# SandeepaInduwaraSamaranayake/SwinVox

Measured on AMD Instinct MI355X. Metric: views/sec fwd+bwd SwinVox-T 224^2, 32^3 voxel, n_views=8, higher is better.
Workload: dtype bf16; 1 GPU; SwinVox-T full pipeline (ResNet50[:layer3] || Swin multi-stage, cross-view attention, decoder, merger, refiner), fwd+2xBCE+bwd, train mode, B=64 samples x V=8 views of 224x224 per GPU; global_batch=64, n_views=8, images_per_gpu=512, parallelism=single GPU, launch=eager (one host launch per kernel, three streams)

## Files before the change

swinvox_amd/csrc/stencil.hip:

```cpp
#include "common.h"
#include <map>
#include <mutex>
#include <type_traits>

namespace sv {

constexpr int TZ = 4, TY = 8, TX = 8;
constexpr int HZ = TZ + 2, HY = TY + 2, HX = TX + 2;
constexpr int HPOS = HZ * HY * HX;
constexpr int NVOX = TZ * TY * TX;
typedef __attribute__((address_space(3))) bf16x4 lds_bf16x4_t;

__device__ __forceinline__ bf16x4 to_bf16x4(float4 v) {
  bf16x4 b;
  b[0] = (__bf16)v.x; b[1] = (__bf16)v.y; b[2] = (__bf16)v.z; b[3] = (__bf16)v.w;
  return b;
}
__device__ __forceinline__ bf16x4 to_bf16x4(bf16x4 v) { return v; }

__device__ __forceinline__ int xcd_first_tile() {
  const int n = gridDim.x, b = blockIdx.x;
  return (n & 7) == 0 ? (b & 7) * (n >> 3) + (b >> 3) : b;
}

struct TileId { int img, z0, y0, x0; };
template <int TZV = TZ>
__device__ __forceinline__ TileId tile_of(int t, int D, int H, int W) {
  const int tz = D / TZV, ty = H / TY, tx = W / TX;
  TileId r;
  r.x0 = (t % tx) * TX; t /= tx; r.y0 = (t % ty) * TY; t /= ty; r.z0 = (t % tz) * TZV; r.img = t / tz;
  return r;
}

template <int G, typename AT, int TZV = TZ, int NTHR = 256>
struct HaloRegs {
  static constexpr int HZV = TZV + 2, HPOSV = HZV * HY * HX;
  static constexpr int C = 16 * G, VPP = C / 4, N = (HPOSV * VPP + NTHR - 1) / NTHR;
  typedef typename std::conditional<G == 1, int, long long>::type OffT;
  typename V4<AT>::type r[N];
  OffT off[N];
  int face[N];
  int lds[N];
  __device__ __forceinline__ void init(int ldx, long long plane, int cin_load, int H, int W, int tid, int pitch = HX) {
#pragma unroll
    for (int k = 0; k < N; ++k) {
      const int i = tid + NTHR * k;
      const int h = i / VPP, v = i - h * VPP;
      const int hx = h % HX; const int t2 = h / HX; const int hy = t2 % HY; const int hz = t2 / HY;
      const int cv = v * 4, pl = plane ? cv / ldx : 0;
      face[k] = (hz == 0 ? 1 : 0) | (hz == HZV - 1 ? 2 : 0) | (hy == 0 ? 4 : 0) | (hy == HY - 1 ? 8 : 0) | (hx == 0 ? 16 : 0) | (hx == HX - 1 ? 32 : 0) |
                ((i < HPOSV * VPP && cv < cin_load) ? 0 : 64);
      off[k] = (OffT)pl * (OffT)plane + (OffT)(((hz * H + hy) * W + hx) * ldx + (cv - pl * ldx));
      lds[k] = ((hz * HY + hy) * pitch + hx) * C + cv;
    }
  }
  __device__ __forceinline__ void load(const AT* __restrict__ x, int ldx, const TileId& t, int D, int H, int W) {
    const int out = (t.z0 == 0 ? 1 : 0) | (t.z0 + TZV == D ? 2 : 0) | (t.y0 == 0 ? 4 : 0) | (t.y0 + TY == H ? 8 : 0) | (t.x0 == 0 ? 16 : 0) | (t.x0 + TX == W ? 32 : 0) | 64;
    const AT* corner = x + ((((long long)t.img * D + t.z0 - 1) * H + t.y0 - 1) * W + t.x0 - 1) * (long long)ldx;
#pragma unroll
    for (int k = 0; k < N; ++k) {
      typename V4<AT>::type q = V4<AT>::zero();
#ifndef SV_ST_PROBE_NOLOAD
      if ((face[k] & out) == 0) q = V4<AT>::load(corner + off[k]);
#endif
      r[k] = q;
    }
  }
  __device__ __forceinline__ void store(__bf16* Xs, int tid) const {
#pragma unroll
    for (int k = 0; k < N; ++k) {
      const int i = tid + NTHR * k;
      if (i < HPOSV * VPP) *reinterpret_cast<bf16x4*>(Xs + lds[k]) = to_bf16x4(r[k]);
    }
  }
};

template <int G, typename AT, int TZV, int NTHR>
struct HaloSliceRegs {
  static constexpr int HZV = TZV + 2, C = 16 * G, VPP = C / 4;
  static constexpr int ZG = G == 1 ? 5 : 2, NGRP = HZV / ZG, GV = ZG * HY * HX * VPP, NP = (GV + NTHR - 1) / NTHR, N = NGRP * NP;
  static_assert(HZV % ZG == 0, "groups of whole z-slices");
  static_assert(HZV * HY * 16 * C < (1 << 20), "LDS offsets (pitch <= 16 positions) take 20 bits");
  typename V4<AT>::type r[N];
  int off[NP], meta[NP];
  long long plane_;
  int gstep_, lstep_;
  __device__ __forceinline__ void init(int ldx, long long plane, int cin_load, int H, int W, int tid, int pitch) {
#pragma unroll
    for (int j = 0; j < NP; ++j) {
      const int i = tid + NTHR * j;
      int h = i / VPP, v = i - h * VPP;
      const int nvp = ldx / 4;
      if (plane && VPP % nvp == 0) {
        const int row = i / (HX * VPP), rem = i - row * (HX * VPP);
        const int pq = rem / (HX * nvp), r2 = rem - pq * (HX * nvp), px = r2 / nvp;
        h = row * HX + px; v = pq * nvp + (r2 - px * nvp);
      }
      const int hx = h % HX; const int t2 = h / HX; const int hy = t2 % HY; const int hz = t2 / HY;
      const int cv = v * 4, pl = plane ? cv / ldx : 0;
      const int fc = (hz == 0 ? 1 : 0) | (hz == ZG - 1 ? 2 : 0) | (hy == 0 ? 4 : 0) | (hy == HY - 1 ? 8 : 0) | (hx == 0 ? 16 : 0) | (hx == HX - 1 ? 32 : 0) |
                     ((i < GV && cv < cin_load) ? 0 : 64);
      const int lo = i < GV ? ((hz * HY + hy) * pitch + hx) * C + cv : 0;
      meta[j] = lo | (fc << 20) | (pl << 27);
      off[j] = ((hz * H + hy) * W + hx) * ldx + (cv - pl * ldx);
    }
    plane_ = plane; gstep_ = ZG * H * W * ldx; lstep_ = ZG * HY * pitch * C;
  }
  __device__ __forceinline__ void load(const AT* __restrict__ x, int ldx, const TileId& t, int D, int H, int W) {
    const int zlo = t.z0 == 0 ? 1 : 0, zhi = t.z0 + TZV == D ? 2 : 0;
    const int yx = (t.y0 == 0 ? 4 : 0) | (t.y0 + TY == H ? 8 : 0) | (t.x0 == 0 ? 16 : 0) | (t.x0 + TX == W ? 32 : 0) | 64;
    const AT* corner = x + ((((long long)t.img * D + t.z0 - 1) * H + t.y0 - 1) * W + t.x0 - 1) * (long long)ldx;
#pragma unroll
    for (int g = 0; g < NGRP; ++g) {
      const int out = (yx | (g == 0 ? zlo : 0) | (g == NGRP - 1 ? zhi : 0)) << 20;
      const AT* cg = corner + (long long)g * gstep_;
#pragma unroll
      for (int j = 0; j < NP; ++j) {
        typename V4<AT>::type q = V4<AT>::zero();
#ifndef SV_ST_PROBE_NOLOAD
        if ((meta[j] & out) == 0) {
          if constexpr (G > 1) q = V4<AT>::load(cg + (long long)((meta[j] >> 27) & 15) * plane_ + off[j]);
          else q = V4<AT>::load(cg + off[j]);
        }
#endif
        r[g * NP + j] = q;
      }
    }
  }
  __device__ __forceinline__ void store(__bf16* Xs, int tid) const {
#pragma unroll
    for (int g = 0; g < NGRP; ++g)
#pragma unroll
      for (int j = 0; j < NP; ++j)
        if ((j + 1) * NTHR <= GV || tid + NTHR * j < GV) *reinterpret_cast<bf16x4*>(Xs + g * lstep_ + (meta[j] & 0xfffff)) = to_bf16x4(r[g * NP + j]);
  }
};

template <typename AT>
struct StencilArgsT {
  const AT* x; int ldx; int cin_load;
  long long x_plane, out_plane;
  const __bf16* w;
  const float* bias; AT* out; int ldc; int col_off; int cout;
  const AT* residual; int ldr;
  double* stats;
  int I, D, H, W, ntiles;
};

template <int G> struct StencilPitch { static constexpr int HXP = G == 1 ? 16 : HX; };
template <int G> struct StencilBrick { static constexpr int TZV = 8, NTHR = TZV * 64; };
template <int G> struct StencilBrickF { static constexpr int TZV = 8, NTHR = TZV * 64; };
template <int G, int NT, typename AT, bool VEC>
__global__ __launch_bounds__(StencilBrickF<G>::NTHR, 2) void stencil3_fwd_kernel(const StencilArgsT<AT> p) {
  constexpr int C = 16 * G, KTOT = 27 * C, KPAD = (KTOT + 31) / 32 * 32, NSTEP = KPAD / 32, HXP = StencilPitch<G>::HXP;
  constexpr int TZV = StencilBrickF<G>::TZV, NTHR = StencilBrickF<G>::NTHR, NW = NTHR / 64;
  __shared__ __attribute__((aligned(16))) char xc[(TZV + 2) * HY * HXP * C * 2];
  __shared__ __attribute__((aligned(16))) __bf16 Ws[NT * 16 * KPAD];
  __shared__ float red[16 * 16 * 2];
  __bf16* Xs = reinterpret_cast<__bf16*>(xc);
  const int tid = threadIdx.x, lane = tid & 63, wave = tid >> 6;
  const int lr = lane & 15, lg = lane >> 4;

  for (int i = tid; i < NT * 16 * KPAD / 8; i += NTHR) {
    const int n = (i * 8) / KPAD, k = (i * 8) - n * KPAD;
    bf16x8 v = VecN<__bf16, 8>::zero();
    if (k < KTOT) v = *reinterpret_cast<const bf16x8*>(p.w + (size_t)n * KTOT + k);
    *reinterpret_cast<bf16x8*>(Ws + n * KPAD + k) = v;
  }
  const int cs4 = (p.cout + 3) & ~3;
  float bias4[NT][4], st1[4] = {0.f, 0.f, 0.f, 0.f}, st2[4] = {0.f, 0.f, 0.f, 0.f};
#pragma unroll
  for (int nt = 0; nt < NT; ++nt)
#pragma unroll
    for (int j = 0; j < 4; ++j) { const int n = nt * 16 + lg * 4 + j; bias4[nt][j] = (p.bias && n < p.cout) ? p.bias[n] : 0.f; }

  HaloRegs<G, AT, TZV, NTHR> hr;
  hr.init(p.ldx, p.x_plane, p.cin_load, p.H, p.W, tid, HXP);
  int tile = xcd_first_tile();
  TileId t = tile_of<TZV>(tile < p.ntiles ? tile : 0, p.D, p.H, p.W);
  if (tile < p.ntiles) { hr.load(p.x, p.ldx, t, p.D, p.H, p.W); hr.store(Xs, tid); }
  __syncthreads();
  const int yy = lr >> 3, xx = lr & 7;
  int toff[NSTEP];
#pragma unroll
  for (int s = 0; s < NSTEP; ++s) {
    const int kb = s * 32 + lg * 8;
    int tap = kb / C; const int c = kb - tap * C;
    if (tap > 26) tap = 26;
    const int dz = tap / 9, dy = (tap - dz * 9) / 3, dx = tap - dz * 9 - dy * 3;
    toff[s] = (((dz * HY + dy) * HXP + dx) * C + c) * 2;
  }
  const char* xrow = xc + ((wave * HY + yy) * HXP + xx) * C * 2;
  const char* wrow = reinterpret_cast<const char*>(Ws) + (lr * KPAD + lg * 8) * 2;
  const int n0 = lg * 4;
  bool colreal[NT][4];
#pragma unroll
  for (int nt = 0; nt < NT; ++nt)
#pragma unroll
    for (int j = 0; j < 4; ++j) colreal[nt][j] = nt * 16 + n0 + j < p.cout;
  for (; tile < p.ntiles; tile += gridDim.x) {
    const int next = tile + gridDim.x;
    TileId tn = t;
    if (next < p.ntiles) { tn = tile_of<TZV>(next, p.D, p.H, p.W); hr.load(p.x, p.ldx, tn, p.D, p.H, p.W); }

    f32x4 acc[4][NT];
#pragma unroll
    for (int mt = 0; mt < 4; ++mt)
#pragma unroll
      for (int nt = 0; nt < NT; ++nt) acc[mt][nt] = (f32x4){0.f, 0.f, 0.f, 0.f};
#ifndef SV_ST_PROBE_NOMMA
#pragma unroll
    for (int s = 0; s < NSTEP; ++s) {
      bf16x8 b[NT];
#pragma unroll
      for (int nt = 0; nt < NT; ++nt) b[nt] = *reinterpret_cast<const bf16x8*>(wrow + nt * 16 * KPAD * 2 + s * 64);
      const char* ap = xrow + toff[s];
#pragma unroll
      for (int mt = 0; mt < 4; ++mt) {
        const bf16x8 a = *reinterpret_cast<const bf16x8*>(ap + mt * (2 * HXP * C * 2));
#pragma unroll
        for (int nt = 0; nt < NT; ++nt) acc[mt][nt] = __builtin_amdgcn_mfma_f32_16x16x32_bf16(b[nt], a, acc[mt][nt], 0, 0, 0);
      }
    }
#endif
    const size_t pos0 = (((size_t)t.img * p.D + t.z0 + wave) * p.H + t.y0 + yy) * p.W + t.x0 + xx;
    if constexpr (VEC) {
#pragma unroll
      for (int nt = 0; nt < NT; ++nt) {
        const int nn = nt * 16 + n0;
        if (nn >= cs4) continue;
        AT* orow; const AT* rrow = nullptr;
        if (p.out_plane) { const int pl = nn / p.ldc; orow = p.out + (size_t)pl * p.out_plane + pos0 * p.ldc + (nn - pl * p.ldc); }
        else orow = p.out + pos0 * p.ldc + p.col_off + nn;
        if (p.residual) rrow = p.residual + pos0 * p.ldr + nn;
#pragma unroll
        for (int mt = 0; mt < 4; ++mt) {
          float v[4];
#pragma unroll
          for (int j = 0; j < 4; ++j) v[j] = colreal[nt][j] ? acc[mt][nt][j] + bias4[nt][j] : 0.f;
          if (NT == 1 && p.stats) {
#pragma unroll
            for (int j = 0; j < 4; ++j) { st1[j] += v[j]; st2[j] += v[j] * v[j]; }
          }
          if (p.residual) {
            const float4 rv = ld4f(rrow + (size_t)mt * 2 * p.W * p.ldr);
            v[0] += rv.x; v[1] += rv.y; v[2] += rv.z; v[3] += rv.w;
          }
#ifdef SV_ST_PROBE_NOSTORE
          if (v[0] == 1234.5f)
#endif
          st4f(orow + (size_t)mt * 2 * p.W * p.ldc, make_float4(v[0], v[1], v[2], v[3]));
        }
      }
    } else {
#pragma unroll
      for (int mt = 0; mt < 4; ++mt) {
        const size_t pos = pos0 + (size_t)mt * 2 * p.W;
#pragma unroll
        for (int nt = 0; nt < NT; ++nt) {
          const int nn = nt * 16 + n0;
#pragma unroll
          for (int j = 0; j < 4; ++j) {
            if (nn + j < p.cout) {
              float r = acc[mt][nt][j] + bias4[nt][j];
              if (NT == 1 && p.stats) { st1[j] += r; st2[j] += r * r; }
              if (p.residual) r += ldf(p.residual + pos * p.ldr + nn + j);
              stf(p.out + pos * p.ldc + p.col_off + nn + j, r);
            }
          }
        }
      }
    }
    t = tn;
    __syncthreads();
    if (next < p.ntiles) hr.store(Xs, tid);
    __syncthreads();
  }
  if (NT == 1 && p.stats) {
#pragma unroll
    for (int j = 0; j < 4; ++j) {
      { st1[j] += dpp_move<0xB1>(st1[j]); st1[j] += dpp_move<0x4E>(st1[j]); st1[j] += dpp_move<0x141>(st1[j]); st1[j] += dpp_move<0x140>(st1[j]);
        st2[j] += dpp_move<0xB1>(st2[j]); st2[j] += dpp_move<0x4E>(st2[j]); st2[j] += dpp_move<0x141>(st2[j]); st2[j] += dpp_move<0x140>(st2[j]); }
    }
    if (lr == 0) {
#pragma unroll
      for (int j = 0; j < 4; ++j) { red[(wave * 16 + lg * 4 + j) * 2] = st1[j]; red[(wave * 16 + lg * 4 + j) * 2 + 1] = st2[j]; }
    }
    __syncthreads();
    if (tid < 16 && tid < p.cout) {
      float a = 0.f, b = 0.f;
#pragma unroll
      for (int w = 0; w < NW; ++w) { a += red[(w * 16 + tid) * 2]; b += red[(w * 16 + tid) * 2 + 1]; }
      double* st = p.stats + (size_t)(blockIdx.x % SV_BN_SLOTS) * 2 * p.cout;
      atomicAdd(st + tid, (double)a);
      atomicAdd(st + p.cout + tid, (double)b);
    }
  }
}

template <typename AT>
struct StencilWArgsT {
  const AT* x; int ldx; int cin_load;
  long long x_plane;
  const AT* dy; int lddy; int cout_load;
  float* dw;
  float* ws;
  float* dbias;
  int cout, cin;
  int c_stride, c_valid;
  int I, D, H, W, ntiles;
};

constexpr int WG_SLOTS = 16;
__global__ __launch_bounds__(256) void stencil_wgrad_fold_kernel(const float* __restrict__ ws, float* __restrict__ dw, int n) {
  const int i = blockIdx.x * 256 + threadIdx.x;
  if (i >= n) return;
  float a = 0.f;
#pragma unroll
  for (int sl = 0; sl < WG_SLOTS; ++sl) a += ws[(size_t)sl * n + i];
  dw[i] += a;
}

template <int G, typename AT>
__global__ __launch_bounds__(StencilBrick<G>::NTHR, 2) void stencil3_wgrad_kernel(const StencilWArgsT<AT> p) {
  constexpr int C = 16 * G, TZV = StencilBrick<G>::TZV, NTHR = StencilBrick<G>::NTHR, NW = NTHR / 64, NTAPW = (27 + NW - 1) / NW;
  constexpr int HPOSV = (TZV + 2) * HY * HX, NVOXV = TZV * TY * TX;
  __shared__ __attribute__((aligned(16))) __bf16 Xs[HPOSV * C];
  __shared__ __attribute__((aligned(16))) __bf16 Ds[NVOXV * 16];
  __shared__ float bred[NTHR / 16 * 16];
  const int tid = threadIdx.x, lane = tid & 63, wave = tid >> 6;
  const int lr = lane & 15, lg = lane >> 4, q = lr >> 2, pp = lr & 3;
  const int ntap = (27 - wave + NW - 1) / NW;
  f32x4 acc[NTAPW][G];
#pragma unroll
  for (int i = 0; i < NTAPW; ++i)
#pragma unroll
    for (int gg = 0; gg < G; ++gg) acc[i][gg] = (f32x4){0.f, 0.f, 0.f, 0.f};
  float bsum = 0.f;

  HaloRegs<G, AT, TZV, NTHR> hr;
  hr.init(p.ldx, p.x_plane, p.cin_load, p.H, p.W, tid);
  typename V4<AT>::type dr[4];
  auto load_dy = [&](const TileId& t) {
#pragma unroll
    for (int k = 0; k < 4; ++k) {
      const int i = tid + NTHR * k;
      const int v = i >> 2, c4 = i & 3;
      const int xx = v % TX; const int t2 = v / TX; const int yy = t2 % TY; const int zz = t2 / TY;
      typename V4<AT>::type qv = V4<AT>::zero();
      if (c4 * 4 < p.cout_load)
        qv = V4<AT>::load(p.dy + ((((size_t)t.img * p.D + t.z0 + zz) * p.H + t.y0 + yy) * p.W + t.x0 + xx) * (size_t)p.lddy + c4 * 4);
      dr[k] = qv;
    }
  };
  auto store_dy = [&]() {
#pragma unroll
    for (int k = 0; k < 4; ++k) *reinterpret_cast<bf16x4*>(Ds + (tid + NTHR * k) * 4) = to_bf16x4(dr[k]);
  };

  int tile = xcd_first_tile();
  if (tile < p.ntiles) {
    const TileId t = tile_of<TZV>(tile, p.D, p.H, p.W);
    hr.load(p.x, p.ldx, t, p.D, p.H, p.W); load_dy(t);
    hr.store(Xs, tid); store_dy();
  }
  __syncthreads();
  for (; tile < p.ntiles; tile += gridDim.x) {
    const int next = tile + gridDim.x;
    if (next < p.ntiles) {
      const TileId t = tile_of<TZV>(next, p.D, p.H, p.W);
      hr.load(p.x, p.ldx, t, p.D, p.H, p.W); load_dy(t);
    }
    if (p.dbias) {
      const int c = tid & 15, vg = tid >> 4;
#pragma unroll
      for (int k = 0; k < 16; ++k) bsum += (float)Ds[(vg * 16 + k) * 16 + c];
    }
#pragma unroll 1
    for (int ch = 0; ch < 2 * TZV; ++ch) {
      const int z = ch >> 1, yb = (ch & 1) * 4 + lg;
      const __bf16* asrc = Ds + (((z * TY + yb) * TX) + q) * 16 + pp * 4;
      const bf16x4 alo = __builtin_amdgcn_ds_read_tr16_b64_v4bf16((lds_bf16x4_t*)(asrc));
      const bf16x4 ahi = __builtin_amdgcn_ds_read_tr16_b64_v4bf16((lds_bf16x4_t*)(asrc + 4 * 16));
      const bf16x8 a = __builtin_shufflevector(alo, ahi, 0, 1, 2, 3, 4, 5, 6, 7);
#pragma unroll
      for (int i = 0; i < NTAPW; ++i) {
        if (i < ntap) {
          const int tap = wave + NW * i;
          const int dz = tap / 9, dy = (tap - dz * 9) / 3, dx = tap - dz * 9 - dy * 3;
          const int hb = ((z + dz) * HY + yb + dy) * HX + dx + q;
#pragma unroll
          for (int gg = 0; gg < G; ++gg) {
            const __bf16* bsrc = Xs + hb * C + gg * 16 + pp * 4;
            const bf16x4 blo = __builtin_amdgcn_ds_read_tr16_b64_v4bf16((lds_bf16x4_t*)(bsrc));
            const bf16x4 bhi = __builtin_amdgcn_ds_read_tr16_b64_v4bf16((lds_bf16x4_t*)(bsrc + 4 * C));
            const bf16x8 b = __builtin_shufflevector(blo, bhi, 0, 1, 2, 3, 4, 5, 6, 7);
            acc[i][gg] = __builtin_amdgcn_mfma_f32_16x16x32_bf16(a, b, acc[i][gg], 0, 0, 0);
          }
        }
      }
    }
    __syncthreads();
    if (next < p.ntiles) { hr.store(Xs, tid); store_dy(); }
    __syncthreads();
  }
  if (p.dbias) {
    bred[tid] = bsum;
    __syncthreads();
    if (tid < 16 && tid < p.cout) {
      float a = 0.f;
#pragma unroll
      for (int g2 = 0; g2 < NTHR / 16; ++g2) a += bred[g2 * 16 + tid];
      atomicAdd(p.dbias + tid, a);
    }
  }
  float* dst = p.ws ? p.ws + (size_t)(blockIdx.x % WG_SLOTS) * p.cout * p.cin * 27 : p.dw;
#pragma unroll
  for (int i = 0; i < NTAPW; ++i) {
    if (i < ntap) {
      const int tap = wave + NW * i;
#pragma unroll
      for (int gg = 0; gg < G; ++gg) {
        const int cm = gg * 16 + lr;
        const int grp = cm / p.c_stride, within = cm - grp * p.c_stride;
        const int ci = grp * p.c_valid + within;
        if (within < p.c_valid && ci < p.cin) {
#pragma unroll
          for (int j = 0; j < 4; ++j) {
            const int co = lg * 4 + j;
            if (co < p.cout) atomicAdd(dst + ((size_t)co * p.cin + ci) * 27 + tap, acc[i][gg][j]);
          }
        }
      }
    }
  }
}

#ifdef SV_ST_PROBE_WG_PITCH
constexpr int SWEEP_HXP = SV_ST_PROBE_WG_PITCH;
#else
constexpr int SWEEP_HXP = 12;
#endif
#ifdef SV_ST_PROBE_WG_LA
constexpr int SWEEP_LA = SV_ST_PROBE_WG_LA;
#else
constexpr int SWEEP_LA = 1;
#endif
#ifdef SV_ST_PROBE_WG_NOSWAP
constexpr int SWEEP_DYSWAP = 0;
#else
constexpr int SWEEP_DYSWAP = 4;
#endif
template <int G, typename AT>
__global__ __launch_bounds__(StencilBrick<G>::NTHR, G == 1 && sizeof(AT) == 2 ? 4 : 2) void stencil3_wgrad_sweep_kernel(const StencilWArgsT<AT> p) {
  constexpr int C = 16 * G, TZV = StencilBrick<G>::TZV, NTHR = StencilBrick<G>::NTHR, HXP = SWEEP_HXP;
  constexpr int XELEMS = (TZV + 2) * HY * HXP * C, NVOXV = TZV * TY * TX, LA = SWEEP_LA;
  static_assert(NTHR == 512 && NTHR * 4 == NVOXV * 4, "8 waves: 2 y-halves x 4 pair slots; dy staging = 4 vectors per thread");
  static_assert(4 * 9 * G * 64 * 4 * sizeof(float) <= XELEMS * sizeof(__bf16), "the half-1 accumulators are handed over through the x image");
  __shared__ __attribute__((aligned(16))) __bf16 Xs[XELEMS];
  __shared__ __attribute__((aligned(16))) __bf16 Ds[NVOXV * 16];
  __shared__ float bred[2 * 64];
  const int tid = threadIdx.x, lane = tid & 63, wave = __builtin_amdgcn_readfirstlane(tid >> 6);
  const int lr = lane & 15, lg = lane >> 4, q = lr >> 2, pp = lr & 3;
  const int half = wave & 1, slot = wave >> 1;
  const int p0 = slot ? 1 + 2 * slot : 0;
  const bool three = slot == 0, sums_bias = p.dbias != nullptr && slot == 1;
  f32x4 acc[3][3][G];
#pragma unroll
  for (int pi = 0; pi < 3; ++pi)
#pragma unroll
    for (int dz = 0; dz < 3; ++dz)
#pragma unroll
      for (int gg = 0; gg < G; ++gg) acc[pi][dz][gg] = (f32x4){0.f, 0.f, 0.f, 0.f};
  float bsum = 0.f;

  HaloSliceRegs<G, AT, TZV, NTHR> hr;
  hr.init(p.ldx, p.x_plane, p.cin_load, p.H, p.W, tid, HXP);
  typename V4<AT>::type dr[4];
  const int dv0 = tid >> 2, dc4 = (tid & 3) * 4;
  const int dyoff = (((dv0 / (TY * TX)) * p.H + (dv0 / TX) % TY) * p.W + dv0 % TX) * p.lddy + dc4;
  const int dystep = 2 * p.H * p.W * p.lddy;
  auto load_dy = [&](const TileId& t) {
    const AT* d0 = p.dy + ((((size_t)t.img * p.D + t.z0) * p.H + t.y0) * p.W + t.x0) * (size_t)p.lddy + dyoff;
#pragma unroll
    for (int k = 0; k < 4; ++k) {
      typename V4<AT>::type qv = V4<AT>::zero();
      if (dc4 < p.cout_load) qv = V4<AT>::load(d0 + (size_t)k * dystep);
      dr[k] = qv;
    }
  };
  auto store_dy = [&]() {
#pragma unroll
    for (int k = 0; k < 4; ++k) {
      const int i = tid + NTHR * k;
      const int v = i >> 2, vs = v ^ (((v >> 3) & 1) * SWEEP_DYSWAP);
      *reinterpret_cast<bf16x4*>(Ds + vs * 16 + (i & 3) * 4) = to_bf16x4(dr[k]);
    }
  };
  const int yb = 4 * half + lg;
  const __bf16* xsrc[3];
#pragma unroll
  for (int pi = 0; pi < 3; ++pi) {
    const int pr = (pi < 2 || three) ? p0 + pi : p0;
    const int dy = pr / 3, dx = pr - dy * 3;
    xsrc[pi] = Xs + ((yb + dy) * HXP + dx + q) * C + pp * 4;
  }
  const __bf16* alo_src = Ds + (yb * TX + q + ((yb & 1) ? SWEEP_DYSWAP : 0)) * 16 + pp * 4;
  const __bf16* ahi_src = Ds + (yb * TX + q + 4 - ((yb & 1) ? SWEEP_DYSWAP : 0)) * 16 + pp * 4;

  auto read_dy = [&](int z) {
    const bf16x4 alo = __builtin_amdgcn_ds_read_tr16_b64_v4bf16((lds_bf16x4_t*)(alo_src + z * TY * TX * 16));
    const bf16x4 ahi = __builtin_amdgcn_ds_read_tr16_b64_v4bf16((lds_bf16x4_t*)(ahi_src + z * TY * TX * 16));
    return (bf16x8)__builtin_shufflevector(alo, ahi, 0, 1, 2, 3, 4, 5, 6, 7);
  };
  auto read_x = [&](int s, int pi, int gg) {
    const __bf16* bsrc = xsrc[pi] + s * HY * HXP * C + gg * 16;
    const bf16x4 blo = __builtin_amdgcn_ds_read_tr16_b64_v4bf16((lds_bf16x4_t*)(bsrc));
    const bf16x4 bhi = __builtin_amdgcn_ds_read_tr16_b64_v4bf16((lds_bf16x4_t*)(bsrc + 4 * C));
    return (bf16x8)__builtin_shufflevector(blo, bhi, 0, 1, 2, 3, 4, 5, 6, 7);
  };
  auto sweep = [&](auto PI0, auto NPI) {
    constexpr int pi0 = decltype(PI0)::value, npi = decltype(NPI)::value, NSTEP = (TZV + 2) * npi * G;
    bf16x8 a[4];
    bf16x8 b[LA + 1];
    a[0] = read_dy(0);
#pragma unroll
    for (int n = 0; n < LA; ++n) b[n] = read_x(n / (npi * G), pi0 + (n / G) % npi, n % G);
#pragma unroll
    for (int n = 0; n < NSTEP; ++n) {
      const int s = n / (npi * G), pi = pi0 + (n / G) % npi, gg = n % G;
      if (n % (npi * G) == 0 && s + 1 < TZV) a[(s + 1) % 4] = read_dy(s + 1);
      if (n + LA < NSTEP) b[(n + LA) % (LA + 1)] = read_x((n + LA) / (npi * G), pi0 + ((n + LA) / G) % npi, (n + LA) % G);
      __builtin_amdgcn_sched_barrier(0);
#pragma unroll
      for (int dz = 0; dz < 3; ++dz)
        if (s - dz >= 0 && s - dz < TZV) acc[pi][dz][gg] = __builtin_amdgcn_mfma_f32_16x16x32_bf16(a[(s - dz) % 4], b[n % (LA + 1)], acc[pi][dz][gg], 0, 0, 0);
      __builtin_amdgcn_sched_barrier(0);
    }
  };

  int tile = xcd_first_tile();
  if (tile < p.ntiles) {
    const TileId t = tile_of<TZV>(tile, p.D, p.H, p.W);
    hr.load(p.x, p.ldx, t, p.D, p.H, p.W); load_dy(t);
    hr.store(Xs, tid); store_dy();
  }
  __syncthreads();
  for (; tile < p.ntiles; tile += gridDim.x) {
    const int next = tile + gridDim.x;
    if (next < p.ntiles) {
      const TileId t = tile_of<TZV>(next, p.D, p.H, p.W);
      hr.load(p.x, p.ldx, t, p.D, p.H, p.W); load_dy(t);
    }
#ifndef SV_ST_PROBE_NOMMA
    sweep(std::integral_constant<int, 0>(), std::integral_constant<int, 2>());
    if (three) sweep(std::integral_constant<int, 2>(), std::integral_constant<int, 1>());
    if (sums_bias) {
#pragma unroll
      for (int z = 0; z < TZV; ++z) {
        const bf16x8 a = read_dy(z);
        float t8 = 0.f;
#pragma unroll
        for (int j = 0; j < 8; ++j) t8 += (float)a[j];
        bsum += t8;
      }
    }
#endif
    __syncthreads();
    if (next < p.ntiles) { hr.store(Xs, tid); store_dy(); }
    __syncthreads();
  }
  f32x4* hand = reinterpret_cast<f32x4*>(Xs) + (size_t)slot * 9 * G * 64 + lane;
  if (half == 1) {
#pragma unroll
    for (int pi = 0; pi < 3; ++pi)
#pragma unroll
      for (int dz = 0; dz < 3; ++dz)
#pragma unroll
        for (int gg = 0; gg < G; ++gg) hand[((pi * 3 + dz) * G + gg) * 64] = acc[pi][dz][gg];
  }
  if (sums_bias) bred[half * 64 + lane] = bsum;
  __syncthreads();
  if (p.dbias && tid < 16 && tid < p.cout) {
    float s8 = 0.f;
#pragma unroll
    for (int g2 = 0; g2 < 8; ++g2) s8 += bred[g2 * 16 + tid];
    atomicAdd(p.dbias + tid, s8);
  }
  if (half == 1) return;
  float* dst = p.ws ? p.ws + (size_t)(blockIdx.x % WG_SLOTS) * p.cout * p.cin * 27 : p.dw;
#pragma unroll
  for (int pi = 0; pi < 3; ++pi) {
    if (pi < 2 || three) {
#pragma unroll
      for (int dz = 0; dz < 3; ++dz) {
        const int tap = dz * 9 + p0 + pi;
#pragma unroll
        for (int gg = 0; gg < G; ++gg) {
          const f32x4 o = hand[((pi * 3 + dz) * G + gg) * 64];
          const int cm = gg * 16 + lr;
          const int grp = cm / p.c_stride, within = cm - grp * p.c_stride;
          const int ci = grp * p.c_valid + within;
          if (within < p.c_valid && ci < p.cin) {
#pragma unroll
            for (int j = 0; j < 4; ++j) {
              const int co = lg * 4 + j;
              if (co < p.cout) atomicAdd(dst + ((size_t)co * p.cin + ci) * 27 + tap, acc[pi][dz][gg][j] + o[j]);
            }
          }
        }
      }
    }
  }
}

struct TConv4Args {
  const __bf16* x; const __bf16* w;
  const float* bias; __bf16* out; double* stats; int cout; int I, D, H, W, nbricks;
};
constexpr int T4_JZ = 4, T4_JY = 4, T4_JX = 8, T4_HZ = 6, T4_HY = 6, T4_HX = 10, T4_HPOS = T4_HZ * T4_HY * T4_HX;

__global__ __launch_bounds__(256, 2) void tconv4s2_fwd_kernel(const TConv4Args p) {
  __shared__ __attribute__((aligned(16))) __bf16 Xs[T4_HPOS * 32];
  __shared__ __attribute__((aligned(16))) __bf16 Ws[8 * 8 * 256];
  __shared__ __attribute__((aligned(16))) __bf16 Os[8 * 8 * 16 * 8];
  __shared__ float red[4][16];
  const int tid = threadIdx.x, lane = tid & 63, wave = tid >> 6;
  const int lr = lane & 15, lg = lane >> 4;
  for (int i = tid; i < 8 * 8 * 256 / 8; i += 256) {
    const int c8 = (i & 3) * 8, t = (i >> 2) & 7, co = (i >> 5) & 7, cls = i >> 8;
    const int az = cls >> 2, ay = (cls >> 1) & 1, ax = cls & 1, dz = t >> 2, dy = (t >> 1) & 1, dx = t & 1;
    const int kz = az ? 2 - 2 * dz : 3 - 2 * dz, ky = ay ? 2 - 2 * dy : 3 - 2 * dy, kx = ax ? 2 - 2 * dx : 3 - 2 * dx;
    bf16x8 v = VecN<__bf16, 8>::zero();
    if (co < p.cout) v = *reinterpret_cast<const bf16x8*>(p.w + ((size_t)co * 64 + (kz * 4 + ky) * 4 + kx) * 32 + c8);
    *reinterpret_cast<bf16x8*>(Ws + ((cls * 8 + co) * 256) + t * 32 + c8) = v;
  }
  float bias4[4];
#pragma unroll
  for (int j = 0; j < 4; ++j) bias4[j] = (p.bias && lg < 2 && lg * 4 + j < p.cout) ? p.bias[lg * 4 + j] : 0.f;
  double st1[8], st2[8];
#pragma unroll
  for (int c = 0; c < 8; ++c) { st1[c] = 0.0; st2[c] = 0.0; }
  const int bz = p.D / T4_JZ, by = p.H / T4_JY, bx = p.W / T4_JX;
  __syncthreads();
  for (int brick = blockIdx.x; brick < p.nbricks; brick += gridDim.x) {
    int t = brick;
    const int x0 = (t % bx) * T4_JX; t /= bx;
    const int y0 = (t % by) * T4_JY; t /= by;
    const int z0 = (t % bz) * T4_JZ; const int img = t / bz;
    for (int i = tid; i < T4_HPOS * 4; i += 256) {
      const int h = i >> 2, c8 = (i & 3) * 8;
      const int hx = h % T4_HX; const int t2 = h / T4_HX; const int hy = t2 % T4_HY; const int hz = t2 / T4_HY;
      const int z = z0 - 1 + hz, y = y0 - 1 + hy, xx = x0 - 1 + hx;
      bf16x8 v = VecN<__bf16, 8>::zero();
      if ((unsigned)z < (unsigned)p.D && (unsigned)y < (unsigned)p.H && (unsigned)xx < (unsigned)p.W)
        v = *reinterpret_cast<const bf16x8*>(p.x + ((((size_t)img * p.D + z) * p.H + y) * p.W + xx) * 32 + c8);
      *reinterpret_cast<bf16x8*>(Xs + h * 32 + c8) = v;
    }
    __syncthreads();
    const int yy = lr >> 3, xx = lr & 7;
#pragma unroll 1
    for (int ci = 0; ci < 2; ++ci) {
      const int cls = 2 * wave + ci, az = cls >> 2, ay = (cls >> 1) & 1, ax = cls & 1;
      bf16x8 b[8];
#pragma unroll
      for (int tt = 0; tt < 8; ++tt) {
        b[tt] = VecN<__bf16, 8>::zero();
        if (lr < 8) b[tt] = *reinterpret_cast<const bf16x8*>(Ws + (cls * 8 + lr) * 256 + tt * 32 + lg * 8);
      }
#pragma unroll 2
      for (int g = 0; g < 8; ++g) {
        const int jz = g >> 1, jy = (g & 1) * 2 + yy;
        const int base = ((jz + az) * T4_HY + (jy + ay)) * T4_HX + (xx + ax);
        f32x4 acc = (f32x4){0.f, 0.f, 0.f, 0.f};
#pragma unroll
        for (int tt = 0; tt < 8; ++tt) {
          const int off = ((tt >> 2) * T4_HY + ((tt >> 1) & 1)) * T4_HX + (tt & 1);
          const bf16x8 a = *reinterpret_cast<const bf16x8*>(Xs + (base + off) * 32 + lg * 8);
          acc = __builtin_amdgcn_mfma_f32_16x16x32_bf16(b[tt], a, acc, 0, 0, 0);
        }
        if (lg < 2) {
          bf16x4 o;
#pragma unroll
          for (int j = 0; j < 4; ++j) o[j] = (__bf16)(acc[j] + bias4[j]);
          const int oz = 2 * jz + az, oy = 2 * jy + ay, ox = 2 * xx + ax;
          *reinterpret_cast<bf16x4*>(Os + ((oz * 8 + oy) * 16 + ox) * 8 + lg * 4) = o;
        }
      }
    }
    __syncthreads();
#pragma unroll
    for (int k = 0; k < 4; ++k) {
      const int v = tid + 256 * k;
      const int ox = v & 15, oy = (v >> 4) & 7, oz = v >> 7;
      const bf16x8 o = *reinterpret_cast<const bf16x8*>(Os + v * 8);
      const size_t pos = (((size_t)img * (2 * p.D) + 2 * z0 + oz) * (2 * p.H) + 2 * y0 + oy) * (2 * p.W) + 2 * x0 + ox;
      *reinterpret_cast<bf16x8*>(p.out + pos * 8) = o;
      if (p.stats) {
#pragma unroll
        for (int c = 0; c < 8; ++c) { const double f = (double)(float)o[c]; st1[c] += f; st2[c] += f * f; }
      }
    }
    __syncthreads();
  }
  if (p.stats) {
#pragma unroll
    for (int c = 0; c < 8; ++c) {
      float a = (float)st1[c], b2 = (float)st2[c];
      a = wave_sum(a); b2 = wave_sum(b2);
      if (lane == 0) { red[wave][c] = a; red[wave][8 + c] = b2; }
    }
    __syncthreads();
    if (tid < 16 && (tid & 7) < p.cout) {
      const float v = red[0][tid] + red[1][tid] + red[2][tid] + red[3][tid];
      double* st = p.stats + (size_t)(blockIdx.x % SV_BN_SLOTS) * 2 * p.cout;
      atomicAdd(st + (tid >> 3) * p.cout + (tid & 7), (double)v);
    }
  }
}

}

using namespace sv;

static int resident_per_cu(const void* kernel, int threads = 256) {
  static std::mutex mu;
  static std::map<const void*, int> cache;
  std::lock_guard<std::mutex> lk(mu);
  auto it = cache.find(kernel);
  if (it != cache.end()) return it->second;
  int n = 0;
  if (hipOccupancyMaxActiveBlocksPerMultiprocessor(&n, kernel, threads, 0) != hipSuccess || n < 1) { (void)hipGetLastError(); n = 1; }
  cache[kernel] = n;
  return n;
}

static int stencil_check(int I, int D, int H, int W) {
  SV_REQUIRE(I > 0 && D % 8 == 0 && H % TY == 0 && W % TX == 0, "stencil3: grid %dx%dx%d must be a multiple of the 8x8x8 brick", D, H, W);
  return SV_OK;
}

#define SV_STENCIL_LAUNCH(GG, NTT, VV)                                                                                     \
  do {                                                                                                                    \
    constexpr int nthr = StencilBrickF<GG>::NTHR;                                                                         \
    const int nt_ = I * (D / StencilBrickF<GG>::TZV) * (H / TY) * (W / TX);                                               \
    a.ntiles = nt_;                                                                                                       \
    const int resident = 256 * resident_per_cu((const void*)stencil3_fwd_kernel<GG, NTT, AT, VV>, nthr);                  \
    hipLaunchKernelGGL((stencil3_fwd_kernel<GG, NTT, AT, VV>), dim3(nt_ < resident ? nt_ : resident), dim3(nthr), 0, s, a); \
  } while (0)

extern "C" int sv_stencil3_fwd(const void* x, int ldx, int cin_load, int groups, const void* w_bf16, int ntiles16,
                               const float* bias, void* out, int ldc, int col_off, int cout, const void* residual, int ldr,
                               double* stats, int I, int D, int H, int W, long long x_plane_stride, long long out_plane_stride,
                               int act_dtype, void* stream) {
  SV_REQUIRE(x && w_bf16 && out, "stencil3_fwd: null argument");
  SV_REQUIRE(x_plane_stride >= 0 && out_plane_stride >= 0 && x_plane_stride % 4 == 0 && out_plane_stride % 4 == 0, "stencil3_fwd: bad plane strides");
  SV_REQUIRE(!out_plane_stride || (col_off == 0 && !residual && ldc % 4 == 0 && cout % ldc == 0),
             "stencil3_fwd: planar output needs col_off == 0, no residual and whole planes of ldc (multiple of 4) columns");
  SV_REQUIRE_ACT(act_dtype);
  if (int rc = stencil_check(I, D, H, W)) return rc;
    SV_REQUIRE(cin_load % 4 == 0 && cin_load <= 16 * groups && ldx % 4 == 0 && (x_plane_stride ? cin_load % ldx == 0 : ldx >= cin_load),
             "stencil3_fwd: bad input channels (cin_load=%d ldx=%d groups=%d)", cin_load, ldx, groups);
  SV_REQUIRE(cout > 0 && cout <= 16 * ntiles16 && (out_plane_stride || ldc >= col_off + cout), "stencil3_fwd: bad output window");
  SV_REQUIRE(!stats || ntiles16 == 1, "stencil3_fwd: statistics need a single 16-column tile");
  const uintptr_t amask = act_dtype == SV_BF16 ? 7 : 15;
  SV_REQUIRE(((uintptr_t)x & amask) == 0 && ((uintptr_t)w_bf16 & 15) == 0, "stencil3_fwd: operands must be aligned to 4 elements");
  SV_REQUIRE((ldc & 3) != 0 || (((uintptr_t)out | (uintptr_t)residual) & amask) == 0,
             "stencil3_fwd: out/residual must be aligned to 4 elements when ldc is a multiple of 4");
  const int ntiles = I * (D / TZ) * (H / TY) * (W / TX);
  hipStream_t s = (hipStream_t)stream;
  if (!((groups == 1 && ntiles16 == 1) || (groups == 3 && ntiles16 == 1) || (groups == 1 && ntiles16 == 3))) {
    set_error("stencil3_fwd: unsupported (groups=%d, ntiles16=%d)", groups, ntiles16);
    return SV_ERR_INVALID;
  }
  SV_DISPATCH_ACT(act_dtype,
    const int cs4 = (cout + 3) & ~3;
    const bool vec = out_plane_stride != 0 || ((ldc & 3) == 0 && (col_off & 3) == 0 && col_off + cs4 <= ldc && (!residual || ((ldr & 3) == 0 && cs4 <= ldr)));
    StencilArgsT<AT> a{static_cast<const AT*>(x), ldx, cin_load, x_plane_stride, out_plane_stride, (const __bf16*)w_bf16, bias, static_cast<AT*>(out), ldc, col_off, cout,
                       static_cast<const AT*>(residual), ldr, stats, I, D, H, W, ntiles};
    if (groups == 1 && ntiles16 == 1) { if (vec) SV_STENCIL_LAUNCH(1, 1, true); else SV_STENCIL_LAUNCH(1, 1, false); }
    else if (groups == 3) { if (vec) SV_STENCIL_LAUNCH(3, 1, true); else SV_STENCIL_LAUNCH(3, 1, false); }
    else { if (vec) SV_STENCIL_LAUNCH(1, 3, true); else SV_STENCIL_LAUNCH(1, 3, false); });
  return check_launch("sv_stencil3_fwd");
}

extern "C" size_t sv_stencil3_wgrad_workspace_floats(int cout, int cin) { return (size_t)WG_SLOTS * cout * cin * 27; }

extern "C" int sv_stencil3_wgrad(const void* x, int ldx, int cin_load, int groups, const void* dy, int lddy, int cout_load,
                                 float* dw, float* dbias, float* workspace, int cout, int cin, int c_stride, int c_valid, int I, int D, int H,
                                 int W, long long x_plane_stride, int act_dtype, void* stream) {
  SV_REQUIRE(x && dy && dw, "stencil3_wgrad: null argument");
  SV_REQUIRE(x_plane_stride >= 0 && x_plane_stride % 4 == 0 && (!x_plane_stride || cin_load % ldx == 0), "stencil3_wgrad: bad plane stride");
  SV_REQUIRE_ACT(act_dtype);
  if (int rc = stencil_check(I, D, H, W)) return rc;
  SV_REQUIRE(cin_load % 4 == 0 && cin_load <= 16 * groups && ldx % 4 == 0 && cout_load % 4 == 0 && cout_load <= 16 && lddy % 4 == 0,
             "stencil3_wgrad: bad channel layout");
  SV_REQUIRE(cout > 0 && cout <= 16 && cin > 0 && c_stride > 0 && c_valid > 0, "stencil3_wgrad: bad channel counts");
  SV_REQUIRE((((uintptr_t)x | (uintptr_t)dy) & (act_dtype == SV_BF16 ? 7 : 15)) == 0, "stencil3_wgrad: operands must be aligned to 4 elements");
  SV_REQUIRE(groups == 1 || groups == 3, "stencil3_wgrad: unsupported groups=%d", groups);
    const int ntiles = I * (D / (groups == 3 ? StencilBrick<3>::TZV : StencilBrick<1>::TZV)) * (H / TY) * (W / TX);
  hipStream_t s = (hipStream_t)stream;
  const char* sweep_env = getenv("SV_STENCIL_WGRAD_SWEEP");
  const bool sweep = sweep_env ? atoi(sweep_env) != 0 : true;
  SV_DISPATCH_ACT(act_dtype,
    const void* k1 = sweep ? (const void*)stencil3_wgrad_sweep_kernel<1, AT> : (const void*)stencil3_wgrad_kernel<1, AT>;
    const void* k3 = sweep ? (const void*)stencil3_wgrad_sweep_kernel<3, AT> : (const void*)stencil3_wgrad_kernel<3, AT>;
    const int per_cu = groups == 1 ? resident_per_cu(k1, StencilBrick<1>::NTHR) : resident_per_cu(k3, StencilBrick<3>::NTHR);
    const int resident = 256 * per_cu;
    const int blocks = ntiles < resident ? ntiles : resident;
    StencilWArgsT<AT> a{static_cast<const AT*>(x), ldx, cin_load, x_plane_stride, static_cast<const AT*>(dy), lddy, cout_load, dw, workspace, dbias, cout, cin, c_stride, c_valid,
                        I, D, H, W, ntiles};
    if (groups == 1 && sweep) hipLaunchKernelGGL((stencil3_wgrad_sweep_kernel<1, AT>), dim3(blocks), dim3(StencilBrick<1>::NTHR), 0, s, a);
    else if (groups == 1) hipLaunchKernelGGL((stencil3_wgrad_kernel<1, AT>), dim3(blocks), dim3(StencilBrick<1>::NTHR), 0, s, a);
    else if (sweep) hipLaunchKernelGGL((stencil3_wgrad_sweep_kernel<3, AT>), dim3(blocks), dim3(StencilBrick<3>::NTHR), 0, s, a);
    else hipLaunchKernelGGL((stencil3_wgrad_kernel<3, AT>), dim3(blocks), dim3(StencilBrick<3>::NTHR), 0, s, a););
  if (workspace) hipLaunchKernelGGL(stencil_wgrad_fold_kernel, dim3(cdiv(cout * cin * 27, 256)), dim3(256), 0, s, workspace, dw, cout * cin * 27);
  return check_launch("sv_stencil3_wgrad");
}

extern "C" int sv_tconv4s2_fwd(const void* x, const void* w_packed, const float* bias, void* out, double* stats, int I, int D, int H, int W,
                               int cin, int cout, void* stream) {
  SV_REQUIRE(x && w_packed && out && I > 0, "tconv4s2_fwd: null argument");
  SV_REQUIRE(cin == 32 && cout > 0 && cout <= 8, "tconv4s2_fwd: built for 32 input and <= 8 output channels (got %d -> %d)", cin, cout);
  SV_REQUIRE(D % T4_JZ == 0 && H % T4_JY == 0 && W % T4_JX == 0, "tconv4s2_fwd: input grid %dx%dx%d must be a multiple of the 4x4x8 brick", D, H, W);
  SV_REQUIRE((((uintptr_t)x | (uintptr_t)w_packed | (uintptr_t)out) & 15) == 0, "tconv4s2_fwd: operands must be 16-byte aligned");
  TConv4Args a{static_cast<const __bf16*>(x), static_cast<const __bf16*>(w_packed), bias, static_cast<__bf16*>(out), stats, cout, I, D, H, W,
               I * (D / T4_JZ) * (H / T4_JY) * (W / T4_JX)};
  const int blocks = a.nbricks < 512 ? a.nbricks : 512;
  hipLaunchKernelGGL(tconv4s2_fwd_kernel, dim3(blocks), dim3(256), 0, (hipStream_t)stream, a);
  return check_launch("sv_tconv4s2_fwd");
}
```

Before: 4967 views/s.

## Add z-sweep stencil forward kernel reusing A fragments across three dz weight taps

Adds a dedicated forward kernel for the 16->16 channel 3x3x3 stencil layers. Each A fragment loaded from LDS for a z-slice is multiplied against all three dz weight slices and accumulated into the matching output planes. The A and weight reads are software-pipelined with a configurable lookahead and scheduling barriers around the MFMAs. It becomes the default path (an env var can disable it) and aims to cut redundant LDS reads of halo slices, at the cost of more registers and a larger weight tile in LDS.

```diff
diff --git a/swinvox_amd/csrc/stencil.hip b/swinvox_amd/csrc/stencil.hip
--- a/swinvox_amd/csrc/stencil.hip
+++ b/swinvox_amd/csrc/stencil.hip
@@ -281,6 +281,161 @@
     for (int j = 0; j < 4; ++j) {
       { st1[j] += dpp_move<0xB1>(st1[j]); st1[j] += dpp_move<0x4E>(st1[j]); st1[j] += dpp_move<0x141>(st1[j]); st1[j] += dpp_move<0x140>(st1[j]);
         st2[j] += dpp_move<0xB1>(st2[j]); st2[j] += dpp_move<0x4E>(st2[j]); st2[j] += dpp_move<0x141>(st2[j]); st2[j] += dpp_move<0x140>(st2[j]); }
+    }
+    if (lr == 0) {
+#pragma unroll
+      for (int j = 0; j < 4; ++j) { red[(wave * 16 + lg * 4 + j) * 2] = st1[j]; red[(wave * 16 + lg * 4 + j) * 2 + 1] = st2[j]; }
+    }
+    __syncthreads();
+    if (tid < 16 && tid < p.cout) {
+      float a = 0.f, b = 0.f;
+#pragma unroll
+      for (int w = 0; w < NW; ++w) { a += red[(w * 16 + tid) * 2]; b += red[(w * 16 + tid) * 2 + 1]; }
+      double* st = p.stats + (size_t)(blockIdx.x % SV_BN_SLOTS) * 2 * p.cout;
+      atomicAdd(st + tid, (double)a);
+      atomicAdd(st + p.cout + tid, (double)b);
+    }
+  }
+}
+
+#ifdef SV_ST_PROBE_FWD_LA
+constexpr int FWD_SWEEP_LA = SV_ST_PROBE_FWD_LA;
+#else
+constexpr int FWD_SWEEP_LA = 3;
+#endif
+template <int G, int NT, typename AT, bool VEC>
+__global__ __launch_bounds__(StencilBrickF<G>::NTHR, 4) void stencil3_fwd_sweep_kernel(const StencilArgsT<AT> p) {
+  static_assert(G == 1 && NT == 1, "the sweep serves the 16 -> 16 channel layers; G = 3 and NT = 3 keep stencil3_fwd_kernel");
+  constexpr int C = 16, HXP = StencilPitch<G>::HXP, TZV = StencilBrickF<G>::TZV, NTHR = StencilBrickF<G>::NTHR, NW = NTHR / 64;
+  constexpr int KPL = 9 * C, KP = (KPL + 31) / 32 * 32, NSTEP = KP / 32, WP = 3 * KP + 16;
+  constexpr int SLICE = HY * HXP * C * 2, LA = FWD_SWEEP_LA, NU = NSTEP * 6;
+  static_assert(TZV == 8 && NW == 8, "8 waves: 4 M-tiles x 2 z-halves of an 8 x 8 x 8 brick");
+  __shared__ __attribute__((aligned(16))) char xc[(TZV + 2) * SLICE];
+  __shared__ __attribute__((aligned(16))) __bf16 Ws[16 * WP];
+  __shared__ float red[NW * 16 * 2];
+  __bf16* Xs = reinterpret_cast<__bf16*>(xc);
+  const int tid = threadIdx.x, lane = tid & 63, wave = __builtin_amdgcn_readfirstlane(tid >> 6);
+  const int lr = lane & 15, lg = lane >> 4;
+  const int mt = wave & 3, zh = wave >> 2;
+
+  for (int i = tid; i < 16 * 3 * (KP / 8); i += NTHR) {
+    const int n = i / (3 * (KP / 8)), v = i - n * (3 * (KP / 8)), dz = v / (KP / 8), kk = (v - dz * (KP / 8)) * 8;
+    bf16x8 q = VecN<__bf16, 8>::zero();
+    if (kk < KPL) q = *reinterpret_cast<const bf16x8*>(p.w + (size_t)n * 27 * C + dz * KPL + kk);
+    *reinterpret_cast<bf16x8*>(Ws + n * WP + dz * KP + kk) = q;
+  }
+  const int cs4 = (p.cout + 3) & ~3;
+  const int n0 = lg * 4;
+  float bias4[4], st1[4] = {0.f, 0.f, 0.f, 0.f}, st2[4] = {0.f, 0.f, 0.f, 0.f};
+  bool colreal[4];
+#pragma unroll
+  for (int j = 0; j < 4; ++j) { colreal[j] = n0 + j < p.cout; bias4[j] = (p.bias && colreal[j]) ? p.bias[n0 + j] : 0.f; }
+
+  HaloSliceRegs<G, AT, TZV, NTHR> hr;
+  hr.init(p.ldx, p.x_plane, p.cin_load, p.H, p.W, tid, HXP);
+  int tile = xcd_first_tile();
+  TileId t = tile_of<TZV>(tile < p.ntiles ? tile : 0, p.D, p.H, p.W);
+  if (tile < p.ntiles) { hr.load(p.x, p.ldx, t, p.D, p.H, p.W); hr.store(Xs, tid); }
+  __syncthreads();
+  const int yy = lr >> 3, xx = lr & 7;
+  const char* abase[NSTEP];
+#pragma unroll
+  for (int s = 0; s < NSTEP; ++s) {
+    const int kb = s * 32 + lg * 8;
+    int tp = kb / C; const int c = kb - tp * C;
+    if (tp > 8) tp = 8;
+    const int dy = tp / 3, dx = tp - dy * 3;
+    abase[s] = xc + (((4 * zh * HY + 2 * mt + yy + dy) * HXP + xx + dx) * C + c) * 2;
+  }
+  const char* wrow = reinterpret_cast<const char*>(Ws) + (lr * WP + lg * 8) * 2;
+  auto read_w = [&](int s, int dz) { return *reinterpret_cast<const bf16x8*>(wrow + (dz * KP + s * 32) * 2); };
+  auto read_a = [&](int s, int hh) { return *reinterpret_cast<const bf16x8*>(abase[s] + hh * SLICE); };
+  for (; tile < p.ntiles; tile += gridDim.x) {
+    const int next = tile + gridDim.x;
+    TileId tn = t;
+    if (next < p.ntiles) { tn = tile_of<TZV>(next, p.D, p.H, p.W); hr.load(p.x, p.ldx, tn, p.D, p.H, p.W); }
+
+    f32x4 acc[4];
+#pragma unroll
+    for (int j = 0; j < 4; ++j) acc[j] = (f32x4){0.f, 0.f, 0.f, 0.f};
+#ifndef SV_ST_PROBE_NOMMA
+    {
+      bf16x8 wf[3], a[LA + 1];
+#pragma unroll
+      for (int dz = 0; dz < 3; ++dz) wf[dz] = read_w(0, dz);
+#pragma unroll
+      for (int n = 0; n < LA; ++n) a[n] = read_a(n / 6, n % 6);
+#pragma unroll
+      for (int n = 0; n < NU; ++n) {
+        const int s = n / 6, hh = n % 6;
+        if (hh == 4 && s + 1 < NSTEP) wf[0] = read_w(s + 1, 0);
+        if (hh == 5 && s + 1 < NSTEP) wf[1] = read_w(s + 1, 1);
+        if (hh == 0 && s > 0) wf[2] = read_w(s, 2);
+        if (n + LA < NU) a[(n + LA) % (LA + 1)] = read_a((n + LA) / 6, (n + LA) % 6);
+        __builtin_amdgcn_sched_barrier(0);
+#pragma unroll
+        for (int dz = 0; dz < 3; ++dz)
+          if (hh - dz >= 0 && hh - dz < 4)
+            acc[hh - dz] = __builtin_amdgcn_mfma_f32_16x16x32_bf16(wf[dz], a[n % (LA + 1)], acc[hh - dz], 0, 0, 0);
+        __builtin_amdgcn_sched_barrier(0);
+      }
+    }
+#endif
+    const size_t pos0 = (((size_t)t.img * p.D + t.z0 + 4 * zh) * p.H + t.y0 + 2 * mt + yy) * p.W + t.x0 + xx;
+    const size_t zstep = (size_t)p.H * p.W;
+    if constexpr (VEC) {
+      if (n0 < cs4) {
+        AT* orow; const AT* rrow = nullptr;
+        if (p.out_plane) { const int pl = n0 / p.ldc; orow = p.out + (size_t)pl * p.out_plane + pos0 * p.ldc + (n0 - pl * p.ldc); }
+        else orow = p.out + pos0 * p.ldc + p.col_off + n0;
+        if (p.residual) rrow = p.residual + pos0 * p.ldr + n0;
+#pragma unroll
+        for (int j = 0; j < 4; ++j) {
+          float v[4];
+#pragma unroll
+          for (int jj = 0; jj < 4; ++jj) v[jj] = colreal[jj] ? acc[j][jj] + bias4[jj] : 0.f;
+          if (p.stats) {
+#pragma unroll
+            for (int jj = 0; jj < 4; ++jj) { st1[jj] += v[jj]; st2[jj] += v[jj] * v[jj]; }
+          }
+          if (p.residual) {
+            const float4 rv = ld4f(rrow + j * zstep * p.ldr);
+            v[0] += rv.x; v[1] += rv.y; v[2] += rv.z; v[3] += rv.w;
+          }
+#ifdef SV_ST_PROBE_NOSTORE
+          if (v[0] == 1234.5f)
+#endif
+          st4f(orow + j * zstep * p.ldc, make_float4(v[0], v[1], v[2], v[3]));
+        }
+      }
+    } else {
+#pragma unroll
+      for (int j = 0; j < 4; ++j) {
+        const size_t pos = pos0 + j * zstep;
+#pragma unroll
+        for (int jj = 0; jj < 4; ++jj) {
+          if (n0 + jj < p.cout) {
+            float r = acc[j][jj] + bias4[jj];
+            if (p.stats) { st1[jj] += r; st2[jj] += r * r; }
+            if (p.residual) r += ldf(p.residual + pos * p.ldr + n0 + jj);
+#ifdef SV_ST_PROBE_NOSTORE
+            if (r == 1234.5f)
+#endif
+            stf(p.out + pos * p.ldc + p.col_off + n0 + jj, r);
+          }
+        }
+      }
+    }
+    t = tn;
+    __syncthreads();
+    if (next < p.ntiles) hr.store(Xs, tid);
+    __syncthreads();
+  }
+  if (p.stats) {
+#pragma unroll
+    for (int j = 0; j < 4; ++j) {
+      st1[j] += dpp_move<0xB1>(st1[j]); st1[j] += dpp_move<0x4E>(st1[j]); st1[j] += dpp_move<0x141>(st1[j]); st1[j] += dpp_move<0x140>(st1[j]);
+      st2[j] += dpp_move<0xB1>(st2[j]); st2[j] += dpp_move<0x4E>(st2[j]); st2[j] += dpp_move<0x141>(st2[j]); st2[j] += dpp_move<0x140>(st2[j]);
     }
     if (lr == 0) {
 #pragma unroll
@@ -747,6 +902,14 @@
     a.ntiles = nt_;                                                                                                       \
     const int resident = 256 * resident_per_cu((const void*)stencil3_fwd_kernel<GG, NTT, AT, VV>, nthr);                  \
     hipLaunchKernelGGL((stencil3_fwd_kernel<GG, NTT, AT, VV>), dim3(nt_ < resident ? nt_ : resident), dim3(nthr), 0, s, a); \
+  } while (0)
+#define SV_STENCIL_SWEEP_LAUNCH(VV)                                                                                        \
+  do {                                                                                                                    \
+    constexpr int nthr = StencilBrickF<1>::NTHR;                                                                          \
+    const int nt_ = I * (D / StencilBrickF<1>::TZV) * (H / TY) * (W / TX);                                                \
+    a.ntiles = nt_;                                                                                                       \
+    const int resident = 256 * resident_per_cu((const void*)stencil3_fwd_sweep_kernel<1, 1, AT, VV>, nthr);               \
+    hipLaunchKernelGGL((stencil3_fwd_sweep_kernel<1, 1, AT, VV>), dim3(nt_ < resident ? nt_ : resident), dim3(nthr), 0, s, a); \
   } while (0)
 
 extern "C" int sv_stencil3_fwd(const void* x, int ldx, int cin_load, int groups, const void* w_bf16, int ntiles16,
@@ -773,12 +936,15 @@
     set_error("stencil3_fwd: unsupported (groups=%d, ntiles16=%d)", groups, ntiles16);
     return SV_ERR_INVALID;
   }
+  const char* sweep_env = getenv("SV_STENCIL_FWD_SWEEP");
+  const bool sweep = sweep_env ? atoi(sweep_env) != 0 : true;
   SV_DISPATCH_ACT(act_dtype,
     const int cs4 = (cout + 3) & ~3;
     const bool vec = out_plane_stride != 0 || ((ldc & 3) == 0 && (col_off & 3) == 0 && col_off + cs4 <= ldc && (!residual || ((ldr & 3) == 0 && cs4 <= ldr)));
     StencilArgsT<AT> a{static_cast<const AT*>(x), ldx, cin_load, x_plane_stride, out_plane_stride, (const __bf16*)w_bf16, bias, static_cast<AT*>(out), ldc, col_off, cout,
                        static_cast<const AT*>(residual), ldr, stats, I, D, H, W, ntiles};
-    if (groups == 1 && ntiles16 == 1) { if (vec) SV_STENCIL_LAUNCH(1, 1, true); else SV_STENCIL_LAUNCH(1, 1, false); }
+    if (groups == 1 && ntiles16 == 1 && sweep) { if (vec) SV_STENCIL_SWEEP_LAUNCH(true); else SV_STENCIL_SWEEP_LAUNCH(false); }
+    else if (groups == 1 && ntiles16 == 1) { if (vec) SV_STENCIL_LAUNCH(1, 1, true); else SV_STENCIL_LAUNCH(1, 1, false); }
     else if (groups == 3) { if (vec) SV_STENCIL_LAUNCH(3, 1, true); else SV_STENCIL_LAUNCH(3, 1, false); }
     else { if (vec) SV_STENCIL_LAUNCH(1, 3, true); else SV_STENCIL_LAUNCH(1, 3, false); });
   return check_launch("sv_stencil3_fwd");
```

Result: no change. 4997 views/s (median of 6 runs) (+0.6%).
